# LuoweiZhou/VLP

Measured on AMD Instinct MI355X. Metric: samples/sec/node (COCO 100-region, seq64, bs64xN) fp16, higher is better.
Workload: dtype f16; 1 GPU; COCO Captions fine-tune shape: BERT-base 12L, 100 regions x 2048-d, seq_len 64 (L=167), bs 64/GPU, fwd+bwd+FP16 FusedAdam, dropout 0.1, dynamic loss scale; global_batch=64, parallelism=dp1, batch_pool=8, skipped_steps=0, rccl_ranks=1, optimizer=replicated, first_leg_packed=False

## Files before the change

vlp_amd/csrc/gemm_nt.h:

```cpp
#pragma once
#include "common.h"

struct GemmNtParams {
    const f16* X; int64_t ldx;
    const f16* W; int64_t ldw;
    f16* Y; int64_t ldy;
    const f16* bias;
    const f16* residual; int64_t ldr;
    f16* preact; int64_t ldp;
    const f16* mulsrc; int64_t ldm;
    int M, N, K;
    int act;
    int mulmode;
    float alpha;
    DropCtx drop;
    const int32_t* row_map;
    int tiles_n;
    int tiles_total;
    int xcd_remap;
#ifdef VLP_NT_DEBUG
    int dbg;
#endif
};

DEVFN uint64_t nt_drop_row(const GemmNtParams& p, int m) { return p.row_map ? (uint64_t)(uint32_t)p.row_map[m] : (uint64_t)m; }

int vlp_gemm_nt_ph_launch(GemmNtParams& p, int bn, int mode, hipStream_t s);

int vlp_gemm_nt_k32_launch(GemmNtParams& p, bool sg, hipStream_t s);

int vlp_gemm_nt_wp_launch(GemmNtParams& p, int cfg, bool sg, hipStream_t s);

bool vlp_gemm_nt_ps_eligible(const GemmNtParams& p, bool sg);
int vlp_gemm_nt_ps_launch(GemmNtParams& p, bool sg, hipStream_t s);

int vlp_gemm_nt_fill_params(const vlp_gemm_nt_args* a, GemmNtParams& p);
int vlp_gemm_nt_splitk_launch(GemmNtParams& p, int splits, float* workspace, int64_t workspace_bytes, hipStream_t s);
```

vlp_amd/csrc/gemm_nt.hip:

```cpp
#include "common.h"
#include "gemm_nt.h"
#include "gemm_nt_epilogue.h"

#define BM 128
#define BK 64


#ifdef VLP_NT_DEBUG
__device__ unsigned long long g_nt_trace[4096 * 4];
#define NT_TRACE(slot) do { if (wid == 0 && lane == 0 && blockIdx.x < 4096) g_nt_trace[blockIdx.x * 4 + (slot)] = wall_clock64(); } while (0)
extern "C" int vlp_debug_read_nt_trace(void* dst, int64_t bytes) { return (int)hipMemcpyFromSymbol(dst, HIP_SYMBOL(g_nt_trace), bytes); }
#else
#define NT_TRACE(slot) do { } while (0)
#endif
DEVFN int swz_x(int r) { return r & 7; }
DEVFN int swz_w(int r) { return (((r >> 4) & 3) << 1) | ((r >> 1) & 1); }

template <int VARIANT, int BM_T, int BN_T, bool SG, int NSR = 0, int EPI = 0>
__global__ __launch_bounds__((BM_T / 64) * (BN_T / 64) * 64, (VARIANT == 3 ? (BN_T == 256 ? 4 : BM_T / 128) : ((VARIANT == 2 || BN_T == 256) ? 4 : 2))) void gemm_nt_kernel(GemmNtParams p) {
    extern __shared__ __attribute__((aligned(16))) char smem_raw[];
    f16* smem = reinterpret_cast<f16*>(smem_raw);
    constexpr int WN_ = BN_T / 64;
    constexpr int T = (BM_T / 64) * WN_ * 64;
    constexpr int RPP = T / 8;
// ... 263 lines not shown
                }
                ST8_OUT(p, p.Y + (int64_t)m * p.ldy + ncol0 + 8 * h, o);
            }
        }
        return;
    }
#pragma unroll
    for (int tm = 0; tm < 4; ++tm) {
        const int m = m0 + wm * 64 + 16 * tm + li;
        if (m >= p.M) continue;
        const uint32_t rkey = p.drop.thresh ? drop_rowkey(p.drop, nt_drop_row(p, m)) : 0u;
        float v[16];
#pragma unroll
        for (int tn = 0; tn < 4; ++tn)
#pragma unroll
            for (int r = 0; r < 4; ++r) v[tn * 4 + r] = acc[tm][tn][r] * p.alpha + bias_v[tn * 4 + r];
#pragma unroll
        for (int h = 0; h < 2; ++h)
            nt_epilogue8<SG>(p, m, ncol0 + 8 * h, v + 8 * h, rkey, true);
    }
#ifdef VLP_NT_DEBUG
    NT_TRACE(2);
    asm volatile("s_waitcnt vmcnt(0)" ::: "memory");
    NT_TRACE(3);
#endif
}

int vlp_gemm_nt_fill_params(const vlp_gemm_nt_args* a, GemmNtParams& p) {
    VLP_CHECK_ARG(a != nullptr, "vlp_gemm_nt: null args");
    VLP_CHECK_ARG(a->X && a->W && a->Y, "vlp_gemm_nt: null operand");
    VLP_CHECK_ARG(a->M > 0 && a->N > 0 && a->K > 0, "vlp_gemm_nt: bad shape M=%d N=%d K=%d", a->M, a->N, a->K);
    VLP_CHECK_ARG(a->K % BK == 0, "vlp_gemm_nt: K=%d must be a multiple of %d (pad with vlp_copy2d)", a->K, BK);
    VLP_CHECK_ARG(a->ldx % 8 == 0 && a->ldw % 8 == 0 && a->ldy % 8 == 0, "vlp_gemm_nt: leading dims must be multiples of 8 halfs");
    VLP_CHECK_ARG(a->ldx >= a->K && a->ldw >= a->K, "vlp_gemm_nt: ldx/ldw < K");
    const int n8 = (a->N + 7) / 8 * 8;
    VLP_CHECK_ARG(a->ldy >= n8, "vlp_gemm_nt: ldy=%lld < roundup8(N)=%d", (long long)a->ldy, n8);
    VLP_CHECK_ARG(((uintptr_t)a->X | (uintptr_t)a->W | (uintptr_t)a->Y) % 16 == 0, "vlp_gemm_nt: operands must be 16-byte aligned");
    if (a->residual) VLP_CHECK_ARG(a->ldr % 8 == 0 && a->ldr >= n8 && (uintptr_t)a->residual % 16 == 0, "vlp_gemm_nt: bad residual layout");
    if (a->preact) VLP_CHECK_ARG(a->ldp % 8 == 0 && a->ldp >= n8 && (uintptr_t)a->preact % 16 == 0, "vlp_gemm_nt: bad preact layout");
    if (a->mul_mode != VLP_MUL_NONE)
        VLP_CHECK_ARG(a->mul_src && a->ldm % 8 == 0 && a->ldm >= n8 && (uintptr_t)a->mul_src % 16 == 0, "vlp_gemm_nt: bad mul_src layout");
    if (a->bias) VLP_CHECK_ARG((uintptr_t)a->bias % 16 == 0, "vlp_gemm_nt: bias must be 16-byte aligned");
    VLP_CHECK_ARG(a->act >= VLP_ACT_NONE && a->act <= VLP_ACT_GELU_SAVE_GRAD, "vlp_gemm_nt: bad act %d", a->act);
    VLP_CHECK_ARG(a->act != VLP_ACT_GELU_SAVE_GRAD || a->preact, "vlp_gemm_nt: VLP_ACT_GELU_SAVE_GRAD needs `preact` (receives gelu'(z))");
    VLP_CHECK_ARG(a->mul_mode >= VLP_MUL_NONE && a->mul_mode <= VLP_MUL_PLAIN, "vlp_gemm_nt: bad mul_mode %d", a->mul_mode);
    VLP_CHECK_ARG(a->dropout_p >= 0.f && a->dropout_p < 1.f, "vlp_gemm_nt: bad dropout p");

    p.X = (const f16*)a->X; p.ldx = a->ldx;
    p.W = (const f16*)a->W; p.ldw = a->ldw;
    p.Y = (f16*)a->Y; p.ldy = a->ldy;
    p.bias = (const f16*)a->bias;
    p.residual = (const f16*)a->residual; p.ldr = a->ldr;
    p.preact = (f16*)a->preact; p.ldp = a->ldp;
    p.mulsrc = (const f16*)a->mul_src; p.ldm = a->ldm;
    p.M = a->M; p.N = a->N; p.K = a->K;
    p.act = a->act; p.mulmode = a->mul_mode;
    p.alpha = a->alpha;
    p.drop = make_drop(a->dropout_p, a->seed, a->rng_stream);
    p.row_map = a->row_map;
    p.tiles_n = 0;
    p.xcd_remap = 0;
#ifdef VLP_NT_DEBUG
    { const char* e = getenv("VLP_NT_DEBUG"); p.dbg = e ? atoi(e) : 0; }
#endif
    return VLP_OK;
}

static thread_local int t_last_variant = -1;
extern "C" int vlp_gemm_nt_resolved_variant(void) { return t_last_variant; }

extern "C" int vlp_gemm_nt(const vlp_gemm_nt_args* a, void* stream) {
    VLP_ENTER(a ? a->X : nullptr, "vlp_gemm_nt");
    GemmNtParams p;
    const int frc = vlp_gemm_nt_fill_params(a, p);
    if (frc != VLP_OK) return frc;
    hipStream_t s = (hipStream_t)stream;
#define LAUNCH_NT_(V, BMT, BNT, NBUF, SGV, NSRV)                                                                  \
    do {                                                                                                                \
        const size_t smem = (size_t)(NBUF) * ((BMT) + (BNT)) * BK * sizeof(f16);                                        \
        VLP_ONCE_PER_DEVICE((void)hipFuncSetAttribute((const void*)gemm_nt_kernel<V, BMT, BNT, SGV, NSRV>, hipFuncAttributeMaxDynamicSharedMemorySize, (int)smem));                                                            \
        p.tiles_n = cdiv(a->N, (BNT));                                                                                  \
        hipLaunchKernelGGL((gemm_nt_kernel<V, BMT, BNT, SGV, NSRV>), dim3(cdiv(a->M, (BMT)) * p.tiles_n), dim3(((BMT) / 64) * ((BNT) / 64) * 64), smem, s, p); \
    } while (0)
#define LAUNCH_NT(V, BMT, BNT, NBUF) \
    do { if (sg) LAUNCH_NT_(V, BMT, BNT, NBUF, true, 0); else LAUNCH_NT_(V, BMT, BNT, NBUF, false, 0); } while (0)
#define LAUNCH_RING(BMT, BNT, NSV) \
    do { if (sg) LAUNCH_NT_(3, BMT, BNT, NSV, true, NSV); else LAUNCH_NT_(3, BMT, BNT, NSV, false, NSV); } while (0)
    const bool sg = a->act == VLP_ACT_GELU_SAVE_GRAD;
    int variant = a->variant;
    if ((variant & 256) && !vlp_gemm_nt_ps_eligible(p, sg)) variant = (a->N > 1024) ? 29 : 27;
    if ((variant & 64) && !sg && !nt_epilogue_is_light(p)) variant = (a->N > 1024) ? 29 : 27;
    if (sg && !(variant & 64) && ((variant & 7) == 6 || (variant & 7) == 7)) variant = (a->N > 1024) ? 29 : 27;
    if ((variant & 64) && ((int64_t)p.M * p.ldx >= (1ll << 31) || (int64_t)p.N * p.ldw >= (1ll << 31))) variant = (a->N > 1024) ? 29 : 27;
#ifndef VLP_LAB_BUILD
    if (!(variant & (64 | 256)) && ((variant & 7) == 6 || (variant & 7) == 7 || ((variant & 7) == 5 && (variant & 48) == 48))) variant = (a->N > 1024) ? 29 : 27;
    if ((variant & 64) && !(variant & 256)) {
        const int cfg = (variant & 7) + ((variant & 128) ? 8 : 0);
        if (cfg != 1 && cfg != 5) variant = (a->N > 1024) ? 29 : 27;
    }
#endif
    t_last_variant = variant;
    if (sg) {
        VLP_CHECK_ARG(!a->residual && a->mul_mode == VLP_MUL_NONE && a->dropout_p == 0.f,
                      "vlp_gemm_nt: VLP_ACT_GELU_SAVE_GRAD fuses bias + gelu + derivative only (no residual / multiplier / dropout)");
    }
    p.xcd_remap = (variant & 8) ? 1 : 0;
    if (variant & 256) {
        const int rc = vlp_gemm_nt_ps_launch(p, sg, s);
        if (rc != VLP_OK) return rc;
        VLP_CHECK_LAUNCH("vlp_gemm_nt");
        return VLP_OK;
    }
    if (variant & 64) {
        const int rc = vlp_gemm_nt_wp_launch(p, (variant & 7) + ((variant & 128) ? 8 : 0), sg, s);
        if (rc != VLP_OK) return rc;
        VLP_CHECK_LAUNCH("vlp_gemm_nt");
        return VLP_OK;
    }
    switch (variant & 7) {
#ifdef VLP_LAB_BUILD
        case 6: case 7: {
            const int rc = vlp_gemm_nt_ph_launch(p, (variant & 7) == 6 ? 256 : 128, (variant >> 4) & 3, s);
// ... 14 lines not shown
            if ((variant & 48) == 48) { const int rc = vlp_gemm_nt_k32_launch(p, sg, s); if (rc != VLP_OK) return rc; }
            else
#endif
            if (variant & 16) {
                static const int lean_on = [] { const char* e = getenv("VLP_NT_LEAN_EPI"); return (e && e[0] == '0') ? 0 : 1; }();
                const bool lean = lean_on && !sg && p.act == VLP_ACT_NONE && !p.preact && p.mulmode == VLP_MUL_PLAIN && !p.drop.thresh && !p.residual &&
                                  p.N % 16 == 0 && p.ldm % 8 == 0 && ((uintptr_t)p.mulsrc & 15) == 0;
                if (lean) {
                    const size_t smem = (size_t)2 * (256 + 256) * BK * sizeof(f16);
                    VLP_ONCE_PER_DEVICE((void)hipFuncSetAttribute((const void*)gemm_nt_kernel<3, 256, 256, false, 2, 1>, hipFuncAttributeMaxDynamicSharedMemorySize, (int)smem));
                    p.tiles_n = cdiv(a->N, 256);
                    hipLaunchKernelGGL((gemm_nt_kernel<3, 256, 256, false, 2, 1>), dim3(cdiv(a->M, 256) * p.tiles_n), dim3(1024), smem, s, p);
                } else {
                    LAUNCH_RING(256, 256, 2);
                }
            }
            else LAUNCH_NT(1, 256, 256, 2);
            break;
        default: LAUNCH_NT(1, 128, 128, 2); break;
    }
#undef LAUNCH_RING
#undef LAUNCH_NT
#undef LAUNCH_NT_
    VLP_CHECK_LAUNCH("vlp_gemm_nt");
    return VLP_OK;
}

extern "C" int vlp_gemm_nt_splitk(const vlp_gemm_nt_args* a, int32_t splits, void* workspace, int64_t workspace_bytes, void* stream) {
    VLP_ENTER(a ? a->X : nullptr, "vlp_gemm_nt_splitk");
    GemmNtParams p;
    const int frc = vlp_gemm_nt_fill_params(a, p);
    if (frc != VLP_OK) return frc;
    VLP_CHECK_ARG(a->act != VLP_ACT_GELU_SAVE_GRAD, "vlp_gemm_nt_splitk: VLP_ACT_GELU_SAVE_GRAD is not provided (training-shape kernels only)");
    return vlp_gemm_nt_splitk_launch(p, splits, (float*)workspace, workspace_bytes, (hipStream_t)stream);
}
```

vlp_amd/csrc/gemm_nt_wp.hip:

```cpp
#include <type_traits>

#include "common.h"
#include "gemm_nt.h"
#include "gemm_nt_epilogue.h"

typedef float f32x16 __attribute__((ext_vector_type(16)));

template <int I, int N, class F>
DEVFN void static_for(F&& f) {
    if constexpr (I < N) {
        f(std::integral_constant<int, I>{});
        static_for<I + 1, N>(f);
    }
}
template <int V> using IC = std::integral_constant<int, V>;

DEVFN void glds16_s(const char* sbase, uint32_t voff, uint32_t lds_dst) {
    const uint32_t m0v = __builtin_amdgcn_readfirstlane(lds_dst);
    asm volatile("s_mov_b32 m0, %0\n\ts_nop 0\n\tglobal_load_lds_dwordx4 %1, %2" ::"s"(m0v), "v"(voff), "s"(sbase) : "memory", "m0");
}
#define WP_SCHED() __builtin_amdgcn_sched_barrier(0)
#ifndef WP_DBG
#define WP_DBG 0
#endif

DEVFN int wp_swz(int r) { return (((r >> 4) & 1) << 2) | (((r >> 3) & 1) << 1) | ((r >> 1) & 1); }
DEVFN int wp_swz_w(int R) { return (R >> 1) & 7; }

DEVFN void wp_light_store8(const GemmNtParams& p, int m, int nc, bool ragged, float (&vv)[8], const f16x8& mulv, const f16x8& resv) {
    if (p.preact) {
        f16x8 z;
#pragma unroll
        for (int j = 0; j < 8; ++j) z[j] = (nc + j < p.N) ? (f16)vv[j] : (f16)0.f;
        st8_out<VLP_SS_SAVED>(p.preact + (int64_t)m * p.ldp + nc, z);
#pragma unroll
        for (int j = 0; j < 8; ++j) vv[j] = (float)z[j];
    }
    if (p.act == VLP_ACT_RELU) {
#pragma unroll
        for (int j = 0; j < 8; ++j) vv[j] = fmaxf(vv[j], 0.f);
    }
    if (p.mulmode == VLP_MUL_PLAIN) {
#pragma unroll
        for (int j = 0; j < 8; ++j) vv[j] *= (float)mulv[j];
    } else if (p.mulmode != VLP_MUL_NONE) {
#pragma unroll
        for (int j = 0; j < 8; ++j) vv[j] = ((float)mulv[j] > 0.f) ? vv[j] : 0.f;
    }
    if (p.drop.thresh) drop_mult8(p.drop, drop_rowkey(p.drop, nt_drop_row(p, m)), (uint32_t)nc, vv);
    if (p.residual) {
#pragma unroll
        for (int j = 0; j < 8; ++j) vv[j] += (float)resv[j];
    }
    f16x8 o;
#pragma unroll
    for (int j = 0; j < 8; ++j) o[j] = (!ragged || nc + j < p.N) ? (f16)vv[j] : (f16)0.f;
    st8_out<VLP_SS_NT>(p.Y + (int64_t)m * p.ldy + nc, o);
}

DEVFN void wp_sg_store8(const GemmNtParams& p, int m, int nc, bool ragged, const float (&vv)[8]) {
    f16x8 d, o;
#pragma unroll
    for (int j = 0; j < 8; ++j) {
        float gl, gp;
        gelu_and_grad_f((float)(f16)vv[j], gl, gp);
        o[j] = (f16)gl;
        d[j] = (f16)gp;
    }
    if (ragged) {
#pragma unroll
        for (int j = 0; j < 8; ++j)
            if (nc + j >= p.N) { o[j] = (f16)0.f; d[j] = (f16)0.f; }
    }
    st8_out<VLP_SS_SAVED>(p.preact + (int64_t)m * p.ldp + nc, d);
    st8_out<VLP_SS_NT>(p.Y + (int64_t)m * p.ldy + nc, o);
}

struct WpDma { int kx, sx, kw, sw; bool dox, dow; };

template <int BN_T, int WGM, int WGN, int NSX, int NSW, bool ROLES, bool SPREAD, bool SG, int PB, int LEAD>
__global__ __launch_bounds__(WGM * WGN * 64, WGM * WGN / 4) void gemm_nt_wp_kernel(GemmNtParams p) {
    extern __shared__ __attribute__((aligned(16))) char smem[];
    constexpr int BM = 256, BK_T = 64, S = 4;
    constexpr int NW = WGM * WGN;
    constexpr int WROWS_M = BM / WGM, WROWS_N = BN_T / WGN;
    constexpr int TM = WROWS_M / 32, TN = WROWS_N / 32;
    constexpr int NM = TM * TN;
    constexpr int NR = TM + TN;
    constexpr int ROWB = BK_T * 2;
    constexpr int NIS = ROLES ? NW / 2 : NW;
    constexpr int LPX = BM / 8 / NIS, LPW = BN_T / 8 / NIS;
    constexpr int XBYTES = BM * ROWB, WBYTES = BN_T * ROWB;
    constexpr int WRING = NSX * XBYTES;
    constexpr int NSMAX = NSX > NSW ? NSX : NSW;
    constexpr bool SPX = SPREAD && NSX >= 3, SPW = SPREAD && NSW >= 3;
    static_assert(ROLES || NSX == NSW, "one wave mixing both streams needs equal ring depths");
    static_assert(TN >= 2 && (BM / 8) % NIS == 0 && (BN_T / 8) % NIS == 0, "tile / wave geometry");
    static_assert((NSX - 1) * LPX + (ROLES ? 0 : (NSW - 1) * LPW) <= 63 && (NSW - 1) * LPW <= 63, "vmcnt range");
    static_assert(PB < NM, "PB");
    constexpr int NB = 2 * LEAD;
    static_assert(LEAD == 1 || LEAD == 2, "LEAD");

    const int tid = threadIdx.x;
    const int lane = tid & 63;
    const int wid = __builtin_amdgcn_readfirstlane(tid >> 6);

    auto tile_origin = [&](int t, int& mo, int& no) {
        if (p.xcd_remap) {
            const int nb = p.tiles_total, q = nb >> 3, r = nb & 7, xcd = t & 7, loc = t >> 3;
            t = (xcd < r ? xcd * (q + 1) : r * (q + 1) + (xcd - r) * q) + loc;
        }
        mo = (t / p.tiles_n) * BM;
        no = (t % p.tiles_n) * BN_T;
    };
    int m0, n0;
    tile_origin(blockIdx.x, m0, n0);
    const int nk = p.K / BK_T;
    const uint32_t lds0 = lds_addr_of(smem);
    const char* const xg = reinterpret_cast<const char*>(p.X);
    const char* const wg = reinterpret_cast<const char*>(p.W);

    const bool xrole = ROLES ? (wid < NW / 2) : true;
    const int lw = ROLES ? (xrole ? wid : wid - NW / 2) : wid;
    uint32_t voffx[LPX], voffw[LPW];
    auto set_dma_tile = [&](int mo, int no) {
        const int rb = lane >> 3, pc = lane & 7;
        static_for<0, LPX>([&](auto J) {
            constexpr int j = decltype(J)::value;
            const int r = (lw + NIS * j) * 8 + rb;
            voffx[j] = (uint32_t)min(mo + r, p.M - 1) * (uint32_t)p.ldx * 2u + (uint32_t)((pc ^ wp_swz(r)) << 4);
        });
        static_for<0, LPW>([&](auto J) {
            constexpr int j = decltype(J)::value;
            const int R = (lw + NIS * j) * 8 + rb;
            voffw[j] = (uint32_t)min(no + R, p.N - 1) * (uint32_t)p.ldw * 2u + (uint32_t)((pc ^ wp_swz_w(R)) << 4);
        });
    };
    set_dma_tile(m0, n0);
    auto issue_x = [&](auto J0_, auto J1_, int kt, int slot) {
        if constexpr (WP_DBG & 2) return;
        const uint32_t dst = __builtin_amdgcn_readfirstlane(lds0 + (uint32_t)slot * XBYTES);
        const char* xs = xg + (int64_t)kt * ROWB;
        static_for<decltype(J0_)::value, decltype(J1_)::value>([&](auto J) {
            constexpr int j = decltype(J)::value;
            glds16_s(xs, voffx[j], dst + (uint32_t)(lw + NIS * j) * 1024u);
        });
    };
    auto issue_w = [&](auto J0_, auto J1_, int kt, int slot) {
        if constexpr (WP_DBG & 2) return;
        const uint32_t dst = __builtin_amdgcn_readfirstlane(lds0 + (uint32_t)WRING + (uint32_t)slot * WBYTES);
        const char* ws = wg + (int64_t)kt * ROWB;
        static_for<decltype(J0_)::value, decltype(J1_)::value>([&](auto J) {
            constexpr int j = decltype(J)::value;
            glds16_s(ws, voffw[j], dst + (uint32_t)(lw + NIS * j) * 1024u);
        });
    };

    const int wm = wid / WGN, wn = wid % WGN;
    const int li = lane & 31, hi = lane >> 5;
    const int fsw = wp_swz(li);
    uint32_t xoff[S], woff[S];
    {
        const int rowx = wm * WROWS_M + li;
        const int roww = wn * WROWS_N + 16 * TN * ((li >> 2) & 1) + 4 * (li >> 3) + (li & 3);
#pragma unroll
        for (int s = 0; s < S; ++s) {
            xoff[s] = (uint32_t)(rowx * ROWB + (((2 * s + hi) ^ fsw) << 4));
            woff[s] = (uint32_t)(WRING + roww * ROWB + (((2 * s + hi) ^ fsw) << 4));
        }
    }
    f32x16 acc[TM][TN];
#pragma unroll
    for (int a = 0; a < TM; ++a)
#pragma unroll
        for (int b = 0; b < TN; ++b)
#pragma unroll
            for (int r = 0; r < 16; ++r) acc[a][b][r] = 0.f;
    constexpr int CW = 32 * TN;
    f16x8 xf[NB][TM], wf[NB][TN];
    if constexpr (WP_DBG & 24) {
#pragma unroll
        for (int b = 0; b < NB; ++b) {
#pragma unroll
            for (int t = 0; t < TM; ++t) xf[b][t] = __builtin_bit_cast(f16x8, (u32x4){(uint32_t)lane, 1u, 2u, 3u});
#pragma unroll
            for (int t = 0; t < TN; ++t) wf[b][t] = __builtin_bit_cast(f16x8, (u32x4){(uint32_t)lane, 5u, 6u, 7u});
        }
    }

    auto read_one = [&](auto BUF_, auto Q_, int xs, int ws, auto SS_) {
        constexpr int BUF = decltype(BUF_)::value, q = decltype(Q_)::value, ss = decltype(SS_)::value;
        if constexpr (WP_DBG & 8) return;
        if constexpr (WP_DBG & 16) {
            const uint32_t a = lds0 + (q == 0 ? (uint32_t)xs + xoff[ss] : (q <= TN ? (uint32_t)ws + woff[ss] + (q - 1) * 16 * ROWB : (uint32_t)xs + xoff[ss] + (q - TN) * 32 * ROWB));
            u32x4 junk;
            asm volatile("ds_read_b128 %0, %1" : "=v"(junk) : "v"(a));
            return;
        }
        if constexpr (q == 0) xf[BUF][0] = ld8(reinterpret_cast<const f16*>(smem + xs + xoff[ss]));
        else if constexpr (q <= TN) wf[BUF][q - 1] = ld8(reinterpret_cast<const f16*>(smem + ws + woff[ss] + (q - 1) * 16 * ROWB));
        else xf[BUF][q - TN] = ld8(reinterpret_cast<const f16*>(smem + xs + xoff[ss] + (q - TN) * 32 * ROWB));
    };
    auto mfma_one = [&](auto BUF_, auto K_) {
        constexpr int BUF = decltype(BUF_)::value, k = decltype(K_)::value, tm = k / TN, tn = k % TN;
        if constexpr (WP_DBG & 1) { const f16x8 a_ = wf[BUF][tn], b_ = xf[BUF][tm]; asm volatile("" ::"v"(a_), "v"(b_)); }
        else acc[tm][tn] = __builtin_amdgcn_mfma_f32_32x32x16_f16(wf[BUF][tn], xf[BUF][tm], acc[tm][tn], 0, 0, 0);
    };
    auto step = [&](auto CUR_, auto DST_, auto MODE_, auto NEXTS_, auto WX_, auto WW_, auto GX_, auto GW_, int rxs, int rws, const WpDma& d) {
        constexpr int CUR = decltype(CUR_)::value, MODE = decltype(MODE_)::value, WX = decltype(WX_)::value, WW = decltype(WW_)::value;
        constexpr int GX = decltype(GX_)::value, GW = decltype(GW_)::value;
        constexpr int FIRST = (MODE == 1) ? PB : 0;
        constexpr int SPAN = NM - FIRST;
        constexpr int X0 = GX < 0 ? 0 : (SPX ? GX * LPX / S : 0), X1 = GX < 0 ? 0 : (SPX ? (GX + 1) * LPX / S : (GX == 0 ? LPX : 0));
        constexpr int W0 = GW < 0 ? 0 : (SPW ? GW * LPW / S : 0), W1 = GW < 0 ? 0 : (SPW ? (GW + 1) * LPW / S : (GW == 0 ? LPW : 0));
        constexpr int NGX = X1 - X0, NGW = W1 - W0, NGB = NGX + NGW;
        static_for<0, NM>([&](auto K_) {
            constexpr int k = decltype(K_)::value;
            if constexpr (MODE == 1 && k == PB) {
                WP_SCHED();
                if (ROLES && !xrole) asm volatile("s_waitcnt vmcnt(%0) lgkmcnt(0)" ::"n"(WW) : "memory");
                else asm volatile("s_waitcnt vmcnt(%0) lgkmcnt(0)" ::"n"(WX) : "memory");
                __builtin_amdgcn_s_barrier();
                WP_SCHED();
            }
            mfma_one(CUR_, K_);
            if constexpr (MODE != 2 && k >= FIRST) {
                static_for<0, NR>([&](auto Q_) {
                    constexpr int q = decltype(Q_)::value;
                    constexpr int rslot = (MODE == 1) ? ((FIRST + q < NM) ? FIRST + q : NM - 1) : (q * SPAN) / NR;
                    if constexpr (rslot == k) read_one(DST_, Q_, rxs, rws, NEXTS_);
                });
            }
// ... 134 lines not shown
                    if (m < p.M && ncol_ok && (EVEN || er + ps * RPP < 32)) mulv[ps] = ld8(p.mulsrc + (int64_t)m * p.ldm + nc);
                }
            }
            if (p.residual) {
#pragma unroll
                for (int ps = 0; ps < NPASS; ++ps) {
                    const int m = mb + ps * RPP;
                    if (m < p.M && ncol_ok && (EVEN || er + ps * RPP < 32)) resv[ps] = ld8(p.residual + (int64_t)m * p.ldr + nc);
                }
            }
        }
#pragma unroll
        for (int ps = 0; ps < NPASS; ++ps) {
            const int m = mb + ps * RPP;
            const int erow = EVEN ? er + ps * RPP : min(er + ps * RPP, 31);
            const f32x4 a0 = *reinterpret_cast<const f32x4*>(ebuf + erow * RS + ec * 4);
            const f32x4 a1 = *reinterpret_cast<const f32x4*>(ebuf + erow * RS + ec * 4 + 16);
            if (m >= p.M || !ncol_ok) continue;
            if (!EVEN && er + ps * RPP >= 32) continue;
            float vv[8];
#pragma unroll
            for (int j = 0; j < 4; ++j) { vv[j] = a0[j] * p.alpha + bias_v[j]; vv[4 + j] = a1[j] * p.alpha + bias_v[4 + j]; }
            if constexpr (SG) {
                wp_sg_store8(p, m, nc, ragged, vv);
            } else {
                wp_light_store8(p, m, nc, ragged, vv, mulv[ps], resv[ps]);
            }
        }
    }
}

int vlp_gemm_nt_wp_launch(GemmNtParams& p, int cfg, bool sg, hipStream_t s) {
    VLP_CHECK_ARG(sg || nt_epilogue_is_light(p), "vlp_gemm_nt: the wave-pipelined variants carry bias / ReLU / multiplier / dropout / residual / save-grad GeLU epilogues only");
    VLP_CHECK_ARG((int64_t)p.M * p.ldx < (1ll << 31) && (int64_t)p.N * p.ldw < (1ll << 31), "vlp_gemm_nt: wave-pipelined variants need M*ldx, N*ldw < 2^31");
#define LAUNCH_WP_(BNT, WGM, WGN, NSXV, NSWV, RLS, SPR, SGV, PBV, LDV)                                                                       \
    do {                                                                                                                               \
        const size_t smem = ((size_t)(NSXV) * 256 + (size_t)(NSWV) * (BNT)) * 64 * sizeof(f16);                                        \
        auto kfn = gemm_nt_wp_kernel<BNT, WGM, WGN, NSXV, NSWV, RLS, SPR, SGV, PBV, LDV>;                                                   \
        VLP_ONCE_PER_DEVICE((void)hipFuncSetAttribute((const void*)kfn, hipFuncAttributeMaxDynamicSharedMemorySize, (int)smem));                                                            \
        p.tiles_n = cdiv(p.N, (BNT));                                                                                                  \
        p.tiles_total = cdiv(p.M, 256) * p.tiles_n;                                                                                    \
        hipLaunchKernelGGL(kfn, dim3(p.tiles_total), dim3((WGM) * (WGN) * 64), smem, s, p);                                            \
    } while (0)
#define LAUNCH_WP(BNT, WGM, WGN, NSXV, NSWV, RLS, SPR, PBV, LDV) \
    do { if (sg) LAUNCH_WP_(BNT, WGM, WGN, NSXV, NSWV, RLS, SPR, true, PBV, LDV); else LAUNCH_WP_(BNT, WGM, WGN, NSXV, NSWV, RLS, SPR, false, PBV, LDV); } while (0)
    switch (cfg) {
        case 1: LAUNCH_WP(256, 2, 4, 2, 2, false, false, 2, 1); break;
        case 5: LAUNCH_WP(128, 4, 2, 3, 3, false, true, 0, 1); break;
#ifdef VLP_LAB_BUILD
        case 0: LAUNCH_WP(256, 2, 2, 2, 2, false, false, 4, 1); break;
        case 2: LAUNCH_WP(256, 2, 2, 2, 2, false, false, 4, 2); break;
        case 3: LAUNCH_WP(256, 2, 2, 3, 2, true, true, 4, 2); break;
        case 4: LAUNCH_WP(128, 2, 2, 3, 3, false, true, 2, 1); break;
        case 6: LAUNCH_WP(128, 2, 2, 3, 3, false, true, 2, 2); break;
        case 7: LAUNCH_WP(128, 4, 2, 3, 3, false, true, 0, 2); break;
        case 8: LAUNCH_WP(128, 4, 2, 3, 3, true, true, 0, 1); break;
        case 10: LAUNCH_WP(192, 4, 2, 2, 2, false, false, 2, 1); break;
        default: LAUNCH_WP(128, 4, 2, 4, 2, true, true, 0, 1); break;
#else
        default: return vlp_set_error(VLP_ERR_BAD_ARG, "vlp_gemm_nt: wave-pipelined configuration %d is an investigation variant (library built without -DVLP_LAB_BUILD)", cfg);
#endif
    }
#undef LAUNCH_WP
#undef LAUNCH_WP_
    return VLP_OK;
}
```

vlp_amd/engine.py:

```python
import math
import os
import weakref

import numpy as np
import torch

from . import _lib as K
from . import tuning
from .input_prep import MaskSpec, RawRegions, SparseAnswers

ALIGN = 64
NO_DECAY = ("bias", "LayerNorm.bias", "LayerNorm.weight")
PE_DIM = 1607
PE_PAD = 1664


def _ru(x, m):
    return (x + m - 1) // m * m


def is_no_decay(name):
    return any(nd in name for nd in NO_DECAY)


# ... 277 lines not shown
            ws.update(sel=h(R, H), tz=h(R, H), tg=h(R, H), tln=h(R, H), tstat=(f(R), f(R)), logits=h(R, Vp), dlogits=h(R, Vp),
                      dlT=h(Vp, _ru(R, 64)),
                      lse_ce=f(R), coef=f(R), row_loss=f(R), dtln=h(R, H), dtg=h(R, H), dtz=h(R, H), dsel=h(R, H))
        ws["loss"] = f(260)
        if model.tasks == "vqa2":
            NA = model.num_answers
            NAp = _ru(NA, 64)
            ws.update(NAp=NAp, vq_e=h(B, H), vq_a1=h(B, 2 * H), vq_logits=h(B, NAp), vq_dlogits=h(B, NAp), vq_dz1=h(B, 2 * H), vq_de=h(B, H))
        ws.update(dx=h(M, H), dx_alt=h(M, H), dpre=h(M, H), dpre_d=h(M, H), dz=h(M, I), dctx=h(M, H), dqkv=h(M, 3 * H),
                  delta=f(B, A, L), d_vis_h=h(Mv, H), d_vispe_h=h(Mv, H), dz1v=h(Mv, 2048), dwpe_pad=h(H, PE_PAD), acc32=f(K.embed_bwd_workspace_floats(B, L, Nv, H)))
        ws["dyset"] = [{"dpre2": h(M, H), "dpre2_d": h(M, H), "dpre1": h(M, H), "dpre1_d": h(M, H), "dz": h(M, I), "dqkv": h(M, 3 * H)}
                       for _ in range(2)]
        tn_bytes = max(K.gemm_tn_workspace_bytes(M, I, H), K.gemm_tn_workspace_bytes(Mv, 2048, 2048), K.gemm_tn_workspace_bytes(M, 3 * H, H))
        ws["tn_ws"] = torch.empty(tn_bytes, device=dev, dtype=torch.uint8)
        ws["tn_ws_main"] = torch.empty(max(K.gemm_tn_workspace_bytes(V, _ru(B * max(P, 1), 64), H), 1 << 20), device=dev, dtype=torch.uint8)
        ws["cs_ws"] = torch.empty(max(K.colsum_workspace_bytes(M, I), K.colsum_workspace_bytes(B * max(P, 1), Vp)), device=dev, dtype=torch.uint8)
        ws["ln_ws"] = torch.empty(K.layernorm_bwd_workspace_bytes(max(H, 8)), device=dev, dtype=torch.uint8)
        ws["ln_slot_bytes"] = K.layernorm_bwd_workspace_bytes(max(H, 8))
        ws["ln_slots"] = torch.empty((2 * NL + 1) * ws["ln_slot_bytes"], device=dev, dtype=torch.uint8)
        self._ws[key] = ws
        return ws

    def _shadows(self):
        if self._shadow is not None:
            return self._shadow
        model = self._model()
        cfg = model.config
        H, I, V = cfg.hidden_size, cfg.intermediate_size, cfg.vocab_size
        dev = self.device

        def h(*s):
            return torch.zeros(*s, device=dev, dtype=torch.float16)

        sh = {"layers": [{"qkvT": h(H, 3 * H), "oT": h(H, H), "w1T": h(H, I), "w2T": h(I, H)} for _ in range(cfg.num_hidden_layers)],
              "v2T": h(2048, H)}
        if model.tasks == "vqa2":
            NAp = _ru(model.num_answers, 64)
            sh.update(a2T=h(2 * H, NAp), a0T=h(H, 2 * H))
        else:
            sh.update(tT=h(H, H))
        self._shadow = sh
        return sh

    def _ln_table(self):
        if self._ln_tab is None:
            NL = self._model().config.num_hidden_layers
            rows = []
            for i in range(NL):
                L = "bert.encoder.layer.%d." % i
                for n in ("attention.output.LayerNorm", "output.LayerNorm"):
                    rows.append([self.G(L + n + ".weight").data_ptr(), self.G(L + n + ".bias").data_ptr()])
            rows.append([self.G("bert.embeddings.LayerNorm.weight").data_ptr(), self.G("bert.embeddings.LayerNorm.bias").data_ptr()])
            self._ln_tab = torch.tensor(rows, dtype=torch.int64, device=self.device)
        return self._ln_tab

    def _refresh_shadows(self):
        sh = self._shadows()
        if "batch" not in sh:
            model = self._model()
            cfg = model.config
            H, I, V = cfg.hidden_size, cfg.intermediate_size, cfg.vocab_size
            items = []
            for i, s in enumerate(sh["layers"]):
                L = "bert.encoder.layer.%d." % i
                items.append((self.P(L + "attention.self.query.weight"), H, s["qkvT"], 3 * H, 3 * H, H, 3 * H))
                items.append((self.P(L + "attention.output.dense.weight"), H, s["oT"], H, H, H, H))
                items.append((self.P(L + "intermediate.dense.weight"), H, s["w1T"], I, I, H, I))
                items.append((self.P(L + "output.dense.weight"), I, s["w2T"], H, H, I, H))
            items.append((self.P("vis_embed.2.weight"), 2048, sh["v2T"], H, H, 2048, H))
            if model.tasks == "vqa2":
                NA = model.num_answers
                items.append((self.P("ans_classifier.2.weight"), 2 * H, sh["a2T"], _ru(NA, 64), NA, 2 * H, _ru(NA, 64)))
                items.append((self.P("ans_classifier.0.weight"), H, sh["a0T"], 2 * H, 2 * H, H, 2 * H))
            else:
                items.append((self.P("cls.predictions.transform.dense.weight"), H, sh["tT"], H, H, H, H))
            sh["batch"] = K.make_transpose_batch(items, self.device)
        K.transpose_batched(sh["batch"])

    def _nt_variant(self, x, w, y, M, N, Kd, kw):
        if self.GEMM_NT_VARIANT is not None:
            return self.GEMM_NT_VARIANT
        key = (M, N, Kd)
        v = Engine._nt_choice.get(key)
        if v is not None:
            return v
        if not tuning.AUTOTUNE:
            v = Engine._nt_choice[key] = tuning.nt_variant(M, N, Kd)
            return v
        best = self.NT_CANDIDATES[0]
        if M * N >= 128 * 128 * 4:
            cands = [c for c in (self.NT_CANDIDATES_SKINNY if M <= 1024 else self.NT_CANDIDATES)
                     if not ((c & 7 == 5 and c < 64 or c == 73) and N < 1024)]
            torch.cuda.synchronize()
            best = tuning.best_of(cands, lambda c, i: K.gemm_nt(x, w, y, M, N, Kd, variant=c, **kw), rounds=2, reps=4 if M > 1024 else 12)
        Engine._nt_choice[key] = best
        tuning.remember("nt", M, N, Kd, best)
        return best

    def _nt(self, x, w, y, M, N, Kd, **kw):
        v = self._nt_variant(x, w, y, M, N, Kd, kw)
        if self.prof is not None:
            self._prof_ctr += 1
        if self.prof is None or self._prof_ctr % self.PROF_EVERY:
            K.gemm_nt(x, w, y, M, N, Kd, variant=v, **kw)
            return
        side = self._side if self._side_busy else None
        main = torch.cuda.current_stream()
        if side is not None:
            main.wait_stream(side)
        e0, e1 = torch.cuda.Event(enable_timing=True), torch.cuda.Event(enable_timing=True)
        e0.record()
        K.gemm_nt(x, w, y, M, N, Kd, variant=v, **kw)
        e1.record()
        if side is not None:
            side.wait_stream(main)
        self.prof.append((e0, e1, 2.0 * M * N * Kd))

    def _nt_skinny(self, x, w, y, M, N, Kd, skws, tune_ws=None, **kw):
        if M > 1024 or N > 4096 or Kd < 256:
            return self._nt(x, w, y, M, N, Kd, **kw)
        key = (M, N, Kd)
        ch = Engine._skinny_choice.get(key)
        if ch is None and not tuning.AUTOTUNE:
            ch = Engine._skinny_choice[key] = tuning.skinny_choice(M, N, Kd)
        if ch is None:
            wl = list(tune_ws()) if tune_ws is not None else [w]
            cands = [("v", v) for v in self.NT_CANDIDATES_SKINNY] + [("s", sp) for sp in tuning.SKINNY_SPLITS if Kd // 64 >= sp]

            def launch(c, i):
                ww = wl[i % len(wl)]
                if c[0] == "v":
                    K.gemm_nt(x, ww, y, M, N, Kd, variant=c[1], **kw)
                else:
# ... 816 lines not shown
        def head_tail():
            for fn in head_wgrads:
                fn()
            self._bucket_done(0)
        on_side(head_tail)

        dctx = ws["dctx"]
        scale = 1.0 / math.sqrt(H // A)
        slot_bytes = ws["ln_slot_bytes"]

        def ln_slot(k):
            return ws["ln_slots"][k * slot_bytes:(k + 1) * slot_bytes]

        grouped = M >= 2048
        for i in reversed(range(NL)):
            Ln = "bert.encoder.layer.%d." % i
            a = ws["layers"][i]
            s = sh["layers"][i]
            x_in = ws["layers"][i - 1]["x2"] if i > 0 else ws["x0"]
            ds = ws["dyset"][i & 1]
            if use_side and self._side_done[i & 1] is not None:
                main.wait_event(self._side_done[i & 1])
            dpre = ds["dpre2"]
            K.layernorm_bwd(dx, a["pre2"], self.P(Ln + "output.LayerNorm.weight"), a["st2"][0], a["st2"][1], dpre,
                            self.G(Ln + "output.LayerNorm.weight"), self.G(Ln + "output.LayerNorm.bias"), M, H, ln_slot(2 * i + 1), beta=beta,
                            dx_drop=ds["dpre2_d"] if p > 0 else None, out_drop=(p, seed, 16 * i + 3), defer_reduce=True, row_map=rm)
            dy2 = ds["dpre2_d"] if p > 0 else dpre
            if not grouped:
                on_side(lambda: self._tn(dy2, a["g"], self.G(Ln + "output.dense.weight"), M, H, I, ws, beta, bias=self.G(Ln + "output.dense.bias")))
            self._nt(dy2, s["w2T"], ds["dz"], M, I, H, mul_src=a["z"], mul_mode=K.MUL_PLAIN)
            if not grouped:
                on_side(lambda: self._tn(ds["dz"], a["x1"], self.G(Ln + "intermediate.dense.weight"), M, I, H, ws, beta,
                                         bias=self.G(Ln + "intermediate.dense.bias")))
            self._nt(ds["dz"], s["w1T"], dx, M, H, I, residual=dpre)
            dpre = ds["dpre1"]
            K.layernorm_bwd(dx, a["pre1"], self.P(Ln + "attention.output.LayerNorm.weight"), a["st1"][0], a["st1"][1], dpre,
                            self.G(Ln + "attention.output.LayerNorm.weight"), self.G(Ln + "attention.output.LayerNorm.bias"), M, H, ln_slot(2 * i),
                            beta=beta, dx_drop=ds["dpre1_d"] if p > 0 else None, out_drop=(p, seed, 16 * i + 2), defer_reduce=True, row_map=rm)
            dy1 = ds["dpre1_d"] if p > 0 else dpre
            if not grouped:
                on_side(lambda: self._tn(dy1, a["ctx"], self.G(Ln + "attention.output.dense.weight"), M, H, H, ws, beta,
                                         bias=self.G(Ln + "attention.output.dense.bias")))
            self._nt(dy1, s["oT"], dctx, M, H, H)
            dqkv = ds["dqkv"]
            K.attn_bwd(a["qkv"], ws["maskb"], ws["maskt"], a["ctx"], dctx, a["lse"], dqkv, ws["delta"], B, L, A, scale, dropout_p=pa, seed=seed,
                       rng_stream=16 * i + 1, row_off=ro)

            def last_wgrad():
                if grouped:
                    K.gemm_tn_grouped([
                        (dy2, a["g"], self.G(Ln + "output.dense.weight"), M, H, I, beta, self.G(Ln + "output.dense.bias")),
                        (ds["dz"], a["x1"], self.G(Ln + "intermediate.dense.weight"), M, I, H, beta, self.G(Ln + "intermediate.dense.bias")),
                        (dqkv, x_in, self.G(Ln + "attention.self.query.weight"), M, 3 * H, H, beta, self.G(Ln + "attention.self.query.bias")),
                        (dy1, a["ctx"], self.G(Ln + "attention.output.dense.weight"), M, H, H, beta, self.G(Ln + "attention.output.dense.bias"))])
                else:
                    self._tn(dqkv, x_in, self.G(Ln + "attention.self.query.weight"), M, 3 * H, H, ws, beta,
                             bias=self.G(Ln + "attention.self.query.bias"))
                self._bucket_done(NL - i)
                if use_side:
                    ev = torch.cuda.Event()
                    ev.record(side)
                    self._side_done[i & 1] = ev
            on_side(last_wgrad)
            self._nt(dqkv, s["qkvT"], dx, M, H, 3 * H, residual=dpre)
        if use_side and not grouped:
            main.wait_stream(side)
            self._side_busy = False
        dpre = ws["dpre"]

        K.layernorm_bwd(dx, ws["emb_pre"], self.P(E + "LayerNorm.weight"), ws["stat0"][0], ws["stat0"][1], dpre,
                        self.G(E + "LayerNorm.weight"), self.G(E + "LayerNorm.bias"), M, H, ln_slot(2 * NL), beta=beta, dy_drop=(p, seed, 1000),
                        defer_reduce=True, row_map=rm)
        if rm is not None:
            dense = ws["dx_alt"]
            dense.zero_()
            K.rows_unpack(dpre, rm, M, dense, H)
            dpre = dense

        def embed_bwd(parts):
            args = (ws["vis_h"], ws["vispe_h"], self.G(E + "word_embeddings.weight"), self.G(E + "position_embeddings.weight"),
                    self.G(E + "token_type_embeddings.weight"), ws["d_vis_h"], ws["d_vispe_h"], ws["acc32"], B, L, Nv, H, V, cfg.type_vocab_size)
            kw = dict(drop_p=p, seed=seed, vis_stream=1001, vispe_stream=1002, region_mask=pt[0]["rmask"] if pt is not None else None, parts=parts)
            if parts == 2 and st.pos_ids is not None:
                K.embed_bwd_pos(dpre, input_ids, token_type_ids, st.pos_ids, *args, **kw)
            else:
                K.embed_bwd(dpre, input_ids, token_type_ids, *args, **kw)

        def tables_and_ln_params():
            K.layernorm_bwd_reduce_batched(ws["ln_slots"], self._ln_table(), 2 * NL + 1, M, H, beta=beta)
            embed_bwd(2)
            self._bucket_done(NL + 1)

        embed_bwd(1)
        if use_side:
            self._side_busy = True
        on_side(tables_and_ln_params)
        self._nt(ws["d_vis_h"], sh["v2T"], ws["dz1v"], Mv, 2048, H, mul_src=ws["h1"], mul_mode=K.MUL_RELU_MASK)
# ... 22 lines not shown
```

vlp_amd/tuning.py:

```python
import json
import os

_HERE = os.path.dirname(os.path.abspath(__file__))
TABLE_PATH = os.environ.get("VLP_TUNE_TABLE") or os.path.join(_HERE, "tuned_gfx950.json")
AUTOTUNE = os.environ.get("VLP_AUTOTUNE", "0") == "1"

SKINNY_SPLITS = (2, 3, 4, 6, 8, 12, 16)
TN_SPLIT_CANDIDATES = (0, 2, 3, 4, 5, 6, 7, 8, 10, 12, 14, 16)

_table = None
_found = {}


def _load():
    global _table
    if _table is None:
        _table = {}
        if os.path.exists(TABLE_PATH):
            with open(TABLE_PATH) as f:
                _table = {k: v for k, v in json.load(f).items() if not k.startswith("_")}
    return _table


def _key(kind, M, N, K):
# ... 6 lines not shown
        v = tuple(v)
    return v


def remember(kind, M, N, K, choice):
    _found[_key(kind, M, N, K)] = list(choice) if isinstance(choice, tuple) else choice


def dump(path):
    cur = {}
    if os.path.exists(path):
        with open(path) as f:
            cur = json.load(f)
    cur.update(_found)
    with open(path, "w") as f:
        json.dump(cur, f, indent=0, sort_keys=True)
    return cur


def best_of(candidates, launch, rounds, reps):
    import torch
    score = {c: float("inf") for c in candidates}
    for _ in range(rounds):
        for c in candidates:
            launch(c, 0)
            e0, e1 = torch.cuda.Event(enable_timing=True), torch.cuda.Event(enable_timing=True)
            e0.record()
            for i in range(reps):
                launch(c, i)
            e1.record()
            e1.synchronize()
            score[c] = min(score[c], e0.elapsed_time(e1))
    return min(candidates, key=score.get)


def nt_heuristic(M, N, K):
    if M <= 1024:
        return 1
    if N <= 1024:
        return 77
    if M >= 6144 and 1024 < N <= 2560 and N % 128 == 0 and K > 512:
        return 264
    return 29


def tn_heuristic(M, N, K):
    if M < 1024:
        return (2, 0)
    tiles = ((N + 127) // 128) * ((K + 127) // 128)
    want = max(1, 512 // tiles)
    best = 0
    for s in TN_SPLIT_CANDIDATES:
        if 1 < s <= want and M // s >= 128:
            best = s
    return (2, best)


def skinny_heuristic(M, N, K):
    tiles = ((M + 127) // 128) * ((N + 127) // 128)
    best = None
    for s in SKINNY_SPLITS:
        if s * 2 <= K // 64 and tiles * s <= 512:
            best = s
    if tiles >= 128 or best is None:
        return ("v", 1)
    return ("s", best)
# ... 58 lines not shown
```

Before: 6979 samples/s.

## Read k-major weights directly in backward dgrad GEMMs, dropping transposed weight copies

Adds a k-major W path to the wave-pipelined NT GEMM, using ds_read_tr16_b64 transpose loads from LDS, so backward data-gradient GEMMs can consume the original weight layout. The per-step transposed weight copies for QKV, attention output and FFN1 are no longer produced. This removes the transpose traffic each step, but forces a fixed tile config (variant 64+5, xcd remap) for these GEMMs instead of the tuned choice. The new path also brings a different LDS swizzle and transposed-read cost.

```diff
diff --git a/vlp_amd/csrc/gemm_nt.h b/vlp_amd/csrc/gemm_nt.h
--- a/vlp_amd/csrc/gemm_nt.h
+++ b/vlp_amd/csrc/gemm_nt.h
@@ -18,6 +18,7 @@
     int tiles_n;
     int tiles_total;
     int xcd_remap;
+    int w_kmajor;
 #ifdef VLP_NT_DEBUG
     int dbg;
 #endif
diff --git a/vlp_amd/csrc/gemm_nt.hip b/vlp_amd/csrc/gemm_nt.hip
--- a/vlp_amd/csrc/gemm_nt.hip
+++ b/vlp_amd/csrc/gemm_nt.hip
@@ -319,7 +319,8 @@
     VLP_CHECK_ARG(a->M > 0 && a->N > 0 && a->K > 0, "vlp_gemm_nt: bad shape M=%d N=%d K=%d", a->M, a->N, a->K);
     VLP_CHECK_ARG(a->K % BK == 0, "vlp_gemm_nt: K=%d must be a multiple of %d (pad with vlp_copy2d)", a->K, BK);
     VLP_CHECK_ARG(a->ldx % 8 == 0 && a->ldw % 8 == 0 && a->ldy % 8 == 0, "vlp_gemm_nt: leading dims must be multiples of 8 halfs");
-    VLP_CHECK_ARG(a->ldx >= a->K && a->ldw >= a->K, "vlp_gemm_nt: ldx/ldw < K");
+    const bool kmajor = (a->variant & 512) != 0;
+    VLP_CHECK_ARG(a->ldx >= a->K && a->ldw >= (kmajor ? a->N : a->K), "vlp_gemm_nt: ldx/ldw < K (k-major W: ldw < N)");
     const int n8 = (a->N + 7) / 8 * 8;
     VLP_CHECK_ARG(a->ldy >= n8, "vlp_gemm_nt: ldy=%lld < roundup8(N)=%d", (long long)a->ldy, n8);
     VLP_CHECK_ARG(((uintptr_t)a->X | (uintptr_t)a->W | (uintptr_t)a->Y) % 16 == 0, "vlp_gemm_nt: operands must be 16-byte aligned");
@@ -347,6 +348,7 @@
     p.row_map = a->row_map;
     p.tiles_n = 0;
     p.xcd_remap = 0;
+    p.w_kmajor = kmajor ? 1 : 0;
 #ifdef VLP_NT_DEBUG
     { const char* e = getenv("VLP_NT_DEBUG"); p.dbg = e ? atoi(e) : 0; }
 #endif
@@ -375,6 +377,16 @@
     do { if (sg) LAUNCH_NT_(3, BMT, BNT, NSV, true, NSV); else LAUNCH_NT_(3, BMT, BNT, NSV, false, NSV); } while (0)
     const bool sg = a->act == VLP_ACT_GELU_SAVE_GRAD;
     int variant = a->variant;
+    if (p.w_kmajor) {
+        VLP_CHECK_ARG((variant & ~8) == 512 + 64 + 5 && !sg && nt_epilogue_is_light(p),
+                      "vlp_gemm_nt: k-major W (variant + 512) exists for variant 64 + 5 (+ 8) with a light epilogue only, got variant %d", variant);
+        t_last_variant = variant;
+        p.xcd_remap = (variant & 8) ? 1 : 0;
+        const int rc = vlp_gemm_nt_wp_launch(p, 5, false, s);
+        if (rc != VLP_OK) return rc;
+        VLP_CHECK_LAUNCH("vlp_gemm_nt");
+        return VLP_OK;
+    }
     if ((variant & 256) && !vlp_gemm_nt_ps_eligible(p, sg)) variant = (a->N > 1024) ? 29 : 27;
     if ((variant & 64) && !sg && !nt_epilogue_is_light(p)) variant = (a->N > 1024) ? 29 : 27;
     if (sg && !(variant & 64) && ((variant & 7) == 6 || (variant & 7) == 7)) variant = (a->N > 1024) ? 29 : 27;
@@ -455,5 +467,6 @@
     const int frc = vlp_gemm_nt_fill_params(a, p);
     if (frc != VLP_OK) return frc;
     VLP_CHECK_ARG(a->act != VLP_ACT_GELU_SAVE_GRAD, "vlp_gemm_nt_splitk: VLP_ACT_GELU_SAVE_GRAD is not provided (training-shape kernels only)");
+    VLP_CHECK_ARG(!p.w_kmajor, "vlp_gemm_nt_splitk: k-major W is not provided");
     return vlp_gemm_nt_splitk_launch(p, splits, (float*)workspace, workspace_bytes, (hipStream_t)stream);
 }
diff --git a/vlp_amd/csrc/gemm_nt_wp.hip b/vlp_amd/csrc/gemm_nt_wp.hip
--- a/vlp_amd/csrc/gemm_nt_wp.hip
+++ b/vlp_amd/csrc/gemm_nt_wp.hip
@@ -5,6 +5,12 @@
 #include "gemm_nt_epilogue.h"
 
 typedef float f32x16 __attribute__((ext_vector_type(16)));
+typedef __fp16 fp16x4_t __attribute__((__vector_size__(4 * sizeof(__fp16))));
+
+DEVFN u32x2 wp_tr_read(const char* p) {
+    fp16x4_t t = __builtin_amdgcn_ds_read_tr16_b64_v4f16((__attribute__((address_space(3))) fp16x4_t*)(p));
+    return __builtin_bit_cast(u32x2, t);
+}
 
 template <int I, int N, class F>
 DEVFN void static_for(F&& f) {
@@ -26,6 +32,7 @@
 
 DEVFN int wp_swz(int r) { return (((r >> 4) & 1) << 2) | (((r >> 3) & 1) << 1) | ((r >> 1) & 1); }
 DEVFN int wp_swz_w(int R) { return (R >> 1) & 7; }
+DEVFN int wp_swz_nn(int k) { return ((k & 1) << 1) | ((k & 2) << 2); }
 
 DEVFN void wp_light_store8(const GemmNtParams& p, int m, int nc, bool ragged, float (&vv)[8], const f16x8& mulv, const f16x8& resv) {
     if (p.preact) {
@@ -78,7 +85,7 @@
 
 struct WpDma { int kx, sx, kw, sw; bool dox, dow; };
 
-template <int BN_T, int WGM, int WGN, int NSX, int NSW, bool ROLES, bool SPREAD, bool SG, int PB, int LEAD>
+template <int BN_T, int WGM, int WGN, int NSX, int NSW, bool ROLES, bool SPREAD, bool SG, int PB, int LEAD, bool NN = false>
 __global__ __launch_bounds__(WGM * WGN * 64, WGM * WGN / 4) void gemm_nt_wp_kernel(GemmNtParams p) {
     extern __shared__ __attribute__((aligned(16))) char smem[];
     constexpr int BM = 256, BK_T = 64, S = 4;
@@ -100,6 +107,7 @@
     static_assert(PB < NM, "PB");
     constexpr int NB = 2 * LEAD;
     static_assert(LEAD == 1 || LEAD == 2, "LEAD");
+    static_assert(!NN || (BN_T == 128 && TN == 2), "k-major W: 256-byte stage rows, wave tiles of 64 columns");
 
     const int tid = threadIdx.x;
     const int lane = tid & 63;
@@ -132,8 +140,14 @@
         });
         static_for<0, LPW>([&](auto J) {
             constexpr int j = decltype(J)::value;
-            const int R = (lw + NIS * j) * 8 + rb;
-            voffw[j] = (uint32_t)min(no + R, p.N - 1) * (uint32_t)p.ldw * 2u + (uint32_t)((pc ^ wp_swz_w(R)) << 4);
+            if constexpr (NN) {
+                const int kr = (lw + NIS * j) * 4 + (lane >> 4);
+                const int col = min(no + (((lane & 15) ^ wp_swz_nn(kr)) << 3), p.N - 8);
+                voffw[j] = (uint32_t)kr * (uint32_t)p.ldw * 2u + (uint32_t)col * 2u;
+            } else {
+                const int R = (lw + NIS * j) * 8 + rb;
+                voffw[j] = (uint32_t)min(no + R, p.N - 1) * (uint32_t)p.ldw * 2u + (uint32_t)((pc ^ wp_swz_w(R)) << 4);
+            }
         });
     };
     set_dma_tile(m0, n0);
@@ -149,7 +163,7 @@
     auto issue_w = [&](auto J0_, auto J1_, int kt, int slot) {
         if constexpr (WP_DBG & 2) return;
         const uint32_t dst = __builtin_amdgcn_readfirstlane(lds0 + (uint32_t)WRING + (uint32_t)slot * WBYTES);
-        const char* ws = wg + (int64_t)kt * ROWB;
+        const char* ws = NN ? wg + (int64_t)kt * BK_T * p.ldw * 2 : wg + (int64_t)kt * ROWB;
         static_for<decltype(J0_)::value, decltype(J1_)::value>([&](auto J) {
             constexpr int j = decltype(J)::value;
             glds16_s(ws, voffw[j], dst + (uint32_t)(lw + NIS * j) * 1024u);
@@ -167,6 +181,15 @@
         for (int s = 0; s < S; ++s) {
             xoff[s] = (uint32_t)(rowx * ROWB + (((2 * s + hi) ^ fsw) << 4));
             woff[s] = (uint32_t)(WRING + roww * ROWB + (((2 * s + hi) ^ fsw) << 4));
+        }
+    }
+    uint32_t woffn[TN];
+    if constexpr (NN) {
+        const int q = (lane >> 2) & 3, pp = lane & 3, k0r = 8 * hi + q;
+#pragma unroll
+        for (int t = 0; t < TN; ++t) {
+            const int ch = wn * (WROWS_N / 8) + 4 * (pp & 1) + 2 * t + ((lane >> 4) & 1);
+            woffn[t] = (uint32_t)(WRING + k0r * (BN_T * 2) + ((ch ^ wp_swz_nn(k0r)) << 4) + 8 * (pp >> 1));
         }
     }
     f32x16 acc[TM][TN];
@@ -198,6 +221,11 @@
             return;
         }
         if constexpr (q == 0) xf[BUF][0] = ld8(reinterpret_cast<const f16*>(smem + xs + xoff[ss]));
+        else if constexpr (q <= TN && NN) {
+            const char* a = smem + ws + woffn[q - 1] + ss * 16 * (BN_T * 2);
+            const u32x2 lo = wp_tr_read(a), hi4 = wp_tr_read(a + 4 * (BN_T * 2));
+            wf[BUF][q - 1] = __builtin_bit_cast(f16x8, (u32x4){lo[0], lo[1], hi4[0], hi4[1]});
+        }
         else if constexpr (q <= TN) wf[BUF][q - 1] = ld8(reinterpret_cast<const f16*>(smem + ws + woff[ss] + (q - 1) * 16 * ROWB));
         else xf[BUF][q - TN] = ld8(reinterpret_cast<const f16*>(smem + xs + xoff[ss] + (q - TN) * 32 * ROWB));
     };
@@ -398,7 +426,17 @@
 
 int vlp_gemm_nt_wp_launch(GemmNtParams& p, int cfg, bool sg, hipStream_t s) {
     VLP_CHECK_ARG(sg || nt_epilogue_is_light(p), "vlp_gemm_nt: the wave-pipelined variants carry bias / ReLU / multiplier / dropout / residual / save-grad GeLU epilogues only");
-    VLP_CHECK_ARG((int64_t)p.M * p.ldx < (1ll << 31) && (int64_t)p.N * p.ldw < (1ll << 31), "vlp_gemm_nt: wave-pipelined variants need M*ldx, N*ldw < 2^31");
+    VLP_CHECK_ARG((int64_t)p.M * p.ldx < (1ll << 31) && (int64_t)(p.w_kmajor ? p.K : p.N) * p.ldw < (1ll << 31), "vlp_gemm_nt: wave-pipelined variants need M*ldx, N*ldw < 2^31");
+    if (p.w_kmajor) {
+        VLP_CHECK_ARG(cfg == 5 && !sg && p.N % 8 == 0, "vlp_gemm_nt: k-major W (variant + 512) is carried by variant 64 + 5 with a light epilogue and N %% 8 == 0");
+        const size_t smem = ((size_t)3 * 256 + (size_t)3 * 128) * 64 * sizeof(f16);
+        auto kfn = gemm_nt_wp_kernel<128, 4, 2, 3, 3, false, true, false, 0, 1, true>;
+        VLP_ONCE_PER_DEVICE((void)hipFuncSetAttribute((const void*)kfn, hipFuncAttributeMaxDynamicSharedMemorySize, (int)smem));
+        p.tiles_n = cdiv(p.N, 128);
+        p.tiles_total = cdiv(p.M, 256) * p.tiles_n;
+        hipLaunchKernelGGL(kfn, dim3(p.tiles_total), dim3(512), smem, s, p);
+        return VLP_OK;
+    }
 #define LAUNCH_WP_(BNT, WGM, WGN, NSXV, NSWV, RLS, SPR, SGV, PBV, LDV)                                                                       \
     do {                                                                                                                               \
         const size_t smem = ((size_t)(NSXV) * 256 + (size_t)(NSWV) * (BNT)) * 64 * sizeof(f16);                                        \
diff --git a/vlp_amd/engine.py b/vlp_amd/engine.py
--- a/vlp_amd/engine.py
+++ b/vlp_amd/engine.py
@@ -333,7 +333,7 @@
         def h(*s):
             return torch.zeros(*s, device=dev, dtype=torch.float16)
 
-        sh = {"layers": [{"qkvT": h(H, 3 * H), "oT": h(H, H), "w1T": h(H, I), "w2T": h(I, H)} for _ in range(cfg.num_hidden_layers)],
+        sh = {"layers": [{"w2T": h(I, H)} for _ in range(cfg.num_hidden_layers)],
               "v2T": h(2048, H)}
         if model.tasks == "vqa2":
             NAp = _ru(model.num_answers, 64)
@@ -364,9 +364,6 @@
             items = []
             for i, s in enumerate(sh["layers"]):
                 L = "bert.encoder.layer.%d." % i
-                items.append((self.P(L + "attention.self.query.weight"), H, s["qkvT"], 3 * H, 3 * H, H, 3 * H))
-                items.append((self.P(L + "attention.output.dense.weight"), H, s["oT"], H, H, H, H))
-                items.append((self.P(L + "intermediate.dense.weight"), H, s["w1T"], I, I, H, I))
                 items.append((self.P(L + "output.dense.weight"), I, s["w2T"], H, H, I, H))
             items.append((self.P("vis_embed.2.weight"), 2048, sh["v2T"], H, H, 2048, H))
             if model.tasks == "vqa2":
@@ -398,8 +395,8 @@
         tuning.remember("nt", M, N, Kd, best)
         return best
 
-    def _nt(self, x, w, y, M, N, Kd, **kw):
-        v = self._nt_variant(x, w, y, M, N, Kd, kw)
+    def _nt(self, x, w, y, M, N, Kd, w_kmajor=False, **kw):
+        v = tuning.NT_W_KMAJOR if w_kmajor else self._nt_variant(x, w, y, M, N, Kd, kw)
         if self.prof is not None:
             self._prof_ctr += 1
         if self.prof is None or self._prof_ctr % self.PROF_EVERY:
@@ -1282,7 +1279,7 @@
             if not grouped:
                 on_side(lambda: self._tn(ds["dz"], a["x1"], self.G(Ln + "intermediate.dense.weight"), M, I, H, ws, beta,
                                          bias=self.G(Ln + "intermediate.dense.bias")))
-            self._nt(ds["dz"], s["w1T"], dx, M, H, I, residual=dpre)
+            self._nt(ds["dz"], self.P(Ln + "intermediate.dense.weight"), dx, M, H, I, w_kmajor=True, residual=dpre)
             dpre = ds["dpre1"]
             K.layernorm_bwd(dx, a["pre1"], self.P(Ln + "attention.output.LayerNorm.weight"), a["st1"][0], a["st1"][1], dpre,
                             self.G(Ln + "attention.output.LayerNorm.weight"), self.G(Ln + "attention.output.LayerNorm.bias"), M, H, ln_slot(2 * i),
@@ -1291,7 +1288,7 @@
             if not grouped:
                 on_side(lambda: self._tn(dy1, a["ctx"], self.G(Ln + "attention.output.dense.weight"), M, H, H, ws, beta,
                                          bias=self.G(Ln + "attention.output.dense.bias")))
-            self._nt(dy1, s["oT"], dctx, M, H, H)
+            self._nt(dy1, self.P(Ln + "attention.output.dense.weight"), dctx, M, H, H, w_kmajor=True)
             dqkv = ds["dqkv"]
             K.attn_bwd(a["qkv"], ws["maskb"], ws["maskt"], a["ctx"], dctx, a["lse"], dqkv, ws["delta"], B, L, A, scale, dropout_p=pa, seed=seed,
                        rng_stream=16 * i + 1, row_off=ro)
@@ -1312,7 +1309,7 @@
                     ev.record(side)
                     self._side_done[i & 1] = ev
             on_side(last_wgrad)
-            self._nt(dqkv, s["qkvT"], dx, M, H, 3 * H, residual=dpre)
+            self._nt(dqkv, self.P(Ln + "attention.self.query.weight"), dx, M, H, 3 * H, w_kmajor=True, residual=dpre)
         if use_side and not grouped:
             main.wait_stream(side)
             self._side_busy = False
diff --git a/vlp_amd/tuning.py b/vlp_amd/tuning.py
--- a/vlp_amd/tuning.py
+++ b/vlp_amd/tuning.py
@@ -62,6 +62,9 @@
             e1.synchronize()
             score[c] = min(score[c], e0.elapsed_time(e1))
     return min(candidates, key=score.get)
+
+
+NT_W_KMAJOR = 512 + 77
 
 
 def nt_heuristic(M, N, K):
```

After: 7002 samples/s, median of 6. About the same (+0.3%).
